# smpurkis/PyTorch-Face-Detection-from-Scratch

Hardware: AMD Instinct MI355X
Metric: train imgs/sec (PoolResnet 480^2, bs=256 per GPU) (higher is better)
Workload: dtype f32 (3x3 convs: bf16x3 split MFMA, fp32 accumulate)

## Files before the change

### pytorch-face-detection-from-scratch_amd/csrc/fdet_wgrad3x3_ps.hip

```cpp
#include "fdet_conv3x3_x3.h"
#include "fdet_ps.h"
#include "fdet_ldsdma.h"
#include <algorithm>

using namespace fdet;

typedef __attribute__((address_space(3))) void* lds_void_t;
typedef const __attribute__((address_space(1))) void* glb_void_t;
typedef short s16x4 __attribute__((ext_vector_type(4)));
typedef __attribute__((address_space(3))) s16x4* lds_s16x4_t;
typedef __bf16 bf16x2_t __attribute__((ext_vector_type(2)));
typedef unsigned u32x2_t __attribute__((ext_vector_type(2)));
typedef unsigned u32x4_t __attribute__((ext_vector_type(4)));

namespace {

#ifndef WG_DBG
#define WG_DBG 0
#endif
constexpr int WG_MAXL = 16;
constexpr int XL = 5, ZL = 3;
constexpr int XA = XL * 64 + 4;
constexpr int ZLS = 66;
constexpr int ZA = 212;
constexpr int WG_LDS_UNITS = 16 * XA + 16 * ZA;

struct PsWgArgs {
  const bf16x8* x[WG_MAXL];
  const bf16x8* dz[WG_MAXL];
  float* ws;
  float* wsb;
  int plane, img;
  int lpi, real_lpi, nlines;
  int nslab, lpw;
  unsigned magic_lpi;
};

__device__ __forceinline__ bf16x2_t as_bf16x2(unsigned u) { return __builtin_bit_cast(bf16x2_t, u); }
__device__ __forceinline__ u32x2_t tr2(const char* base, int off) {
  return __builtin_bit_cast(u32x2_t, __builtin_amdgcn_ds_read_tr16_b64_v4i16((lds_s16x4_t)(base + off)));
}
__host__ __device__ constexpr int x_line(int S, int ky, int WP) { return 16 * S + (ky - 1) * WP < 0 ? 0 : (16 * S + (ky - 1) * WP >= 64 ? 2 : 1); }
__host__ __device__ constexpr int x_off(int S, int ky, int WP) {
  return 16 * S + (ky - 1) * WP < 0 ? 16 * S + (ky - 1) * WP + 64 : (16 * S + (ky - 1) * WP >= 64 ? 16 * S + (ky - 1) * WP - 64 : 16 * S + (ky - 1) * WP);
}

template <int WP, bool FL1, bool P16 = false>
__global__ void __launch_bounds__(256, 1)
k_wgrad3x3_ps(const PsWgArgs a) {
  extern __shared__ __attribute__((aligned(16))) char smem[];
  bf16x8* const lds = reinterpret_cast<bf16x8*>(smem);
  const int tid = threadIdx.x, lane = tid & 63;
  const int wid = __builtin_amdgcn_readfirstlane(tid >> 6);
  const int m = wid & 1, j = wid >> 1;
  const int layer = blockIdx.y;
  const bf16x8* __restrict__ gx = a.x[layer];
  const bf16x8* __restrict__ gz = a.dz[layer];
  {
    f32x4* z = reinterpret_cast<f32x4*>(smem);
    for (int t = tid; t < WG_LDS_UNITS; t += 256) z[t] = f32x4{0.f, 0.f, 0.f, 0.f};
  }
  const int i16 = lane & 15, g16 = (lane >> 4) & 1, kh = lane >> 5;
  const int q = i16 >> 2, pp = i16 & 3;
  const int GA = 4 * m + 2 * g16 + (pp >> 1), GB = 4 * j + 2 * g16 + (pp >> 1);
  const int lane_x = (GB * XA + 8 * kh + q) * 16 + (pp & 1) * 8;
  const int lane_z = (16 * XA + GA * ZA + 1 + 8 * kh + q) * 16 + (pp & 1) * 8;
  constexpr int XPL = 8 * XA * 16, ZPL = 8 * ZA * 16;

  const int l0 = blockIdx.x * a.lpw, l1 = min(l0 + a.lpw, a.nlines);
  f32x16 acc[9];
#pragma unroll
  for (int t = 0; t < 9; ++t)
#pragma unroll
    for (int r = 0; r < 16; ++r) acc[t][r] = 0.f;
  float bsum = 0.f;
  const unsigned bsel0 = j == 0 ? 0x3f803f80u : 0u, bsel1 = j == 1 ? 0x3f803f80u : 0u;

  const unsigned lds0 = (unsigned)(size_t)(lds_void_t)smem;
  const unsigned tbytes = (unsigned)((a.nlines / a.lpi) + 2) * (unsigned)a.img * 16u;
  const dma_u32x4 xrs = dma_rsrc(gx - a.img, tbytes), zrs = dma_rsrc(gz - a.img, tbytes);
  const unsigned lane16 = (unsigned)lane * 16u;
#define WG_PIECE(RS, LG, AI, DST)                                                                  \
  {                                                                                                \
    const int lg_ = (LG) + a.lpi;                                                                  \
    const int n_ = (int)__umulhi((unsigned)lg_, a.magic_lpi);                                      \
    const unsigned so_ = (unsigned)(n_ * a.img + ((AI) >> 3) * a.plane + ((AI) & 7) * (a.lpi * 64) + (lg_ - n_ * a.lpi) * 64) * 16u; \
    dma_piece(lds0 + (unsigned)(DST) * 16u, lane16, RS, so_);                                      \
  }
#define WG_ISSUE(LX, SX, LZ, SZ)                                                                   \
  if (!(P16 && wid >= 2)) {                                   \
    _Pragma("unroll") for (int k_ = 0; k_ < 4; ++k_) {                                             \
      const int ai_ = 4 * wid + k_;                                                                \
      WG_PIECE(xrs, LX, ai_, ai_ * XA + (SX) * 64)                                                  \
      WG_PIECE(zrs, LZ, ai_, 16 * XA + ai_ * ZA + (SZ) * ZLS + 1)                                   \
    }                                                                                              \
  }
  __syncthreads();
  int sx = ((l0 - 1) % XL + XL) % XL, sz = l0 % ZL;
#define XS(D) ((sx + (D)) % XL)
  WG_ISSUE(l0 - 1, XS(0), l0, sz)
  WG_ISSUE(l0, XS(1), l0 + 1, (sz + 1) % ZL)
  if (!(P16 && wid >= 2)) {
    _Pragma("unroll") for (int k_ = 0; k_ < 4; ++k_) {
      const int ai_ = 4 * wid + k_;
      WG_PIECE(xrs, l0 + 1, ai_, ai_ * XA + XS(2) * 64)
      WG_PIECE(xrs, l0 + 2, ai_, ai_ * XA + XS(3) * 64)
    }
  }
  asm volatile("s_waitcnt vmcnt(0)" ::: "memory");

  u32x4_t zf[2][3][2], xf[2][3][2];
#define WG_FRAGS(F, S, ZB, XB0, XB1, XB2)                                                          \
  {                                                                                                \
    _Pragma("unroll") for (int k_ = 0; k_ < 3; ++k_)                                               \
      _Pragma("unroll") for (int pl_ = 0; pl_ < (P16 ? 1 : 2); ++pl_)                              \
        _Pragma("unroll") for (int h_ = 0; h_ < 2; ++h_) {                                         \
          const u32x2_t z_ = (WG_DBG & 4) ? u32x2_t{0x3f803f80u + (unsigned)lane, 0x40004000u} : tr2(ZB, pl_ * ZPL + (16 * (S) + 4 * h_ - (k_ - 1)) * 16); \
          zf[F][k_][pl_][2 * h_] = z_[0]; zf[F][k_][pl_][2 * h_ + 1] = z_[1];                      \
          const char* xb_ = x_line((S), k_, WP) == 0 ? XB0 : (x_line((S), k_, WP) == 1 ? XB1 : XB2); \
          const u32x2_t x_ = (WG_DBG & 4) ? u32x2_t{0x3f803f80u, 0x40004000u + (unsigned)lane} : tr2(xb_, pl_ * XPL + (x_off((S), k_, WP) + 4 * h_) * 16); \
          xf[F][k_][pl_][2 * h_] = x_[0]; xf[F][k_][pl_][2 * h_ + 1] = x_[1];                      \
        }                                                                                          \
  }
  int band = l0;
  if (FL1) {
    __builtin_amdgcn_s_barrier();
    const char* zb_ = smem + lane_z + sz * (ZLS * 16);
    const char* xb0 = smem + lane_x + XS(0) * 1024;
    const char* xb1 = smem + lane_x + XS(1) * 1024;
    const char* xb2 = smem + lane_x + XS(2) * 1024;
    WG_FRAGS(0, 0, zb_, xb0, xb1, xb2)
  }
  int row = l0 - (l0 / a.lpi) * a.lpi;
  while (band < l1) {
  const int n_full = row < a.real_lpi ? min(l1 - band, a.real_lpi - row) : 0;
  row += n_full;
  for (const int bend = band + n_full; band < bend; ++band) {
    if (FL1) asm volatile("s_waitcnt vmcnt(0)" ::: "memory");
    else asm volatile("s_waitcnt vmcnt(8)" ::: "memory");
    __builtin_amdgcn_s_barrier();
    if (!(WG_DBG & 1)) WG_ISSUE(band + 3, XS(4), band + 2, (sz + 2) % ZL)
    __builtin_amdgcn_sched_barrier(0);
    {
      const char* zb_ = smem + lane_z + sz * (ZLS * 16);
      const char* xb0 = smem + lane_x + XS(0) * 1024;
      const char* xb1 = smem + lane_x + XS(1) * 1024;
      const char* xb2 = smem + lane_x + XS(2) * 1024;
      const char* zbn = smem + lane_z + ((sz + 1) % ZL) * (ZLS * 16);
      const char* xb3 = smem + lane_x + XS(3) * 1024;
      if (!FL1) {
        WG_FRAGS(0, 0, zb_, xb0, xb1, xb2)
        __builtin_amdgcn_sched_barrier(0);
      }
#pragma unroll
      for (int s = 0; s < 4; ++s) {
        const int F = s & 1;
        if (s < 3) WG_FRAGS(F ^ 1, s + 1, zb_, xb0, xb1, xb2)
        else if (FL1) WG_FRAGS(0, 0, zbn, xb1, xb2, xb3)
#pragma unroll
        for (int ky = 0; ky < 3; ++ky)
#pragma unroll
          for (int kx = 0; kx < 3; ++kx) {
            const int t = ky * 3 + kx;
            const bf16x8 ah = __builtin_bit_cast(bf16x8, zf[F][kx][0]), al = __builtin_bit_cast(bf16x8, zf[F][kx][1]);
            const bf16x8 bh = __builtin_bit_cast(bf16x8, xf[F][ky][0]), bl = __builtin_bit_cast(bf16x8, xf[F][ky][1]);
            if (!(WG_DBG & 2)) {
              if (!P16) {
                acc[t] = __builtin_amdgcn_mfma_f32_32x32x16_bf16(ah, bl, acc[t], 0, 0, 0);
                acc[t] = __builtin_amdgcn_mfma_f32_32x32x16_bf16(al, bh, acc[t], 0, 0, 0);
              }
              acc[t] = __builtin_amdgcn_mfma_f32_32x32x16_bf16(ah, bh, acc[t], 0, 0, 0);
            }
          }
        {
          const bf16x2_t sel = as_bf16x2((s & 1) ? bsel1 : bsel0);
#pragma unroll
          for (int pl = 0; pl < (P16 ? 1 : 2); ++pl) {
            const u32x4_t zv = zf[F][1][pl];
            bsum = __builtin_amdgcn_fdot2_f32_bf16(as_bf16x2(zv[0]), sel, bsum, false);
            bsum = __builtin_amdgcn_fdot2_f32_bf16(as_bf16x2(zv[1]), sel, bsum, false);
            bsum = __builtin_amdgcn_fdot2_f32_bf16(as_bf16x2(zv[2]), sel, bsum, false);
            bsum = __builtin_amdgcn_fdot2_f32_bf16(as_bf16x2(zv[3]), sel, bsum, false);
          }
        }
        if ((s < 3 || FL1) && !P16) {
#pragma unroll
          for (int i = 0; i < 24; ++i) {
            __builtin_amdgcn_sched_group_barrier(0x008, 1, 0);
            __builtin_amdgcn_sched_group_barrier(0x100, 1, 0);
          }
          __builtin_amdgcn_sched_group_barrier(0x008, 3, 0);
        } else if (s < 3 || FL1) {
#pragma unroll
          for (int i = 0; i < 9; ++i) {
            __builtin_amdgcn_sched_group_barrier(0x008, 1, 0);
            if (i < 6) __builtin_amdgcn_sched_group_barrier(0x100, 2, 0);
          }
        }
      }
    }
    sx = (sx + 1) % XL;
    sz = (sz + 1) % ZL;
  }
  if (band < l1 && row >= a.real_lpi) {
    const int n_zero = min(l1 - band, a.lpi - row);
    for (const int bend = band + n_zero; band < bend; ++band) {
      asm volatile("s_waitcnt vmcnt(0)" ::: "memory");
      __builtin_amdgcn_s_barrier();
      if (!(WG_DBG & 1)) WG_ISSUE(band + 3, XS(4), band + 2, (sz + 2) % ZL)
      sx = (sx + 1) % XL;
      sz = (sz + 1) % ZL;
    }
    row += n_zero;
    if (row >= a.lpi) row = 0;
    if (FL1 && band < l1) {
      const char* zb_ = smem + lane_z + sz * (ZLS * 16);
      const char* xb0 = smem + lane_x + XS(0) * 1024;
      const char* xb1 = smem + lane_x + XS(1) * 1024;
      const char* xb2 = smem + lane_x + XS(2) * 1024;
      WG_FRAGS(0, 0, zb_, xb0, xb1, xb2)
    }
  }
  }
  asm volatile("s_waitcnt vmcnt(0)" ::: "memory");
#undef WG_FRAGS
#undef XS
#undef WG_ISSUE
#undef WG_PIECE
  const int l31 = lane & 31, half = lane >> 5;
  const size_t s = (size_t)layer * a.nslab + blockIdx.x;
  float* __restrict__ wsl = a.ws + s * 9 * 64 * 64;
#pragma unroll
  for (int t = 0; t < 9; ++t)
#pragma unroll
    for (int r = 0; r < 16; ++r) {
      const int co = 32 * m + (r & 3) + 8 * (r >> 2) + 4 * half;
      wsl[(t * 64 + co) * 64 + 32 * j + l31] = acc[t][r];
    }
  bsum += __shfl_xor(bsum, 32, 64);
  if (half == 0) a.wsb[(s * 2 + j) * 64 + 32 * m + l31] = bsum;
}

struct PsWgRed { float* dW[WG_MAXL]; float* db[WG_MAXL]; };
__global__ void __launch_bounds__(256)
k_wgrad_ps_reduce(const float* __restrict__ ws, const float* __restrict__ wsb, int nslab, const PsWgRed out) {
  __shared__ float part[256];
  const int layer = blockIdx.y;
  const int el = threadIdx.x & 63, q = threadIdx.x >> 6;
  const bool bias_blk = blockIdx.x == 9 * 64;
  const size_t stride = bias_blk ? 128 : 9 * 4096;
  const float* __restrict__ src = bias_blk ? wsb + (size_t)layer * nslab * 128 + el
                                           : ws + (size_t)layer * nslab * 9 * 4096 + (size_t)blockIdx.x * 64 + el;
  float s = 0.f;
  int k = q;
  for (; k + 28 < nslab; k += 32) {
    float v[8];
#pragma unroll
    for (int u = 0; u < 8; ++u) v[u] = src[(size_t)(k + 4 * u) * stride] + (bias_blk ? src[(size_t)(k + 4 * u) * stride + 64] : 0.f);
#pragma unroll
    for (int u = 0; u < 8; ++u) s += v[u];
  }
  for (; k < nslab; k += 4) s += src[(size_t)k * stride] + (bias_blk ? src[(size_t)k * stride + 64] : 0.f);
  part[threadIdx.x] = s;
  __syncthreads();
  if (q == 0) {
    const float r = ((part[el] + part[64 + el]) + part[128 + el]) + part[192 + el];
    if (bias_blk) {
      out.db[layer][el] = r;
    } else {
      const int e = blockIdx.x * 64 + el;
      const int t = e >> 12, co = (e >> 6) & 63, ci = e & 63;
      out.dW[layer][(co * 64 + ci) * 9 + t] = r;
    }
  }
}

int wg_plan(int L, int N, int H, int W, PsGeo& g, int& nslab, int& lpw) {
  PsStrips sp;
  if (!ps_geo_strips(N, 64, H, W, g, sp) || L < 1 || L > WG_MAXL) return 0;
  const int lpi = g.HP * g.WP / 64;
  const long nlines = (long)g.N * lpi;
  if (nlines + 2 * lpi >= (1 << 20) || (size_t)(g.N + 2) * g.img * 16 >= ((size_t)1 << 32)) return 0;
  nslab = std::max(1, std::min((int)nlines, num_cus() / L));
  lpw = (int)((nlines + nslab - 1) / nslab);
  nslab = (int)((nlines + lpw - 1) / lpw);
  return 1;
}

}

extern "C" size_t fdet_conv3x3_wgrad_ps_ws_bytes(int L, int N, int C, int H, int W) {
  PsGeo g;
  int nslab = 0, lpw = 0;
  if (C != 64 || !wg_plan(L, N, H, W, g, nslab, lpw)) return 0;
  return (size_t)L * nslab * (9 * 4096 + 128) * sizeof(float);
}

namespace {
int wgrad_ps_run(const void* const* h_x, const void* const* h_dz, float* const* h_dW, float* const* h_db, int L, int N, int C,
                 int H, int W, void* ws, size_t ws_bytes, void* stream, bool p16) {
  PsGeo g;
  int nslab = 0, lpw = 0;
  FDET_REQUIRE(h_x && h_dz && h_dW && h_db && ws, "conv3x3_wgrad_ps: null pointer");
  FDET_REQUIRE(C == 64 && wg_plan(L, N, H, W, g, nslab, lpw), "conv3x3_wgrad_ps: unsupported shape (L=%d N=%d C=%d H=%d W=%d)", L, N, C, H, W);
  const size_t need = (size_t)L * nslab * (9 * 4096 + 128) * sizeof(float);
  FDET_REQUIRE(ws_bytes >= need, "conv3x3_wgrad_ps: workspace of %zu bytes needed, %zu given", need, ws_bytes);
  PsWgArgs a;
  PsWgRed red;
  for (int l = 0; l < L; ++l) {
    FDET_REQUIRE(h_x[l] && h_dz[l] && h_dW[l] && h_db[l], "conv3x3_wgrad_ps: null pointer in layer %d", l);
    a.x[l] = reinterpret_cast<const bf16x8*>(h_x[l]);
    a.dz[l] = reinterpret_cast<const bf16x8*>(h_dz[l]);
    red.dW[l] = h_dW[l];
    red.db[l] = h_db[l];
  }
  a.ws = reinterpret_cast<float*>(ws);
  a.wsb = a.ws + (size_t)L * nslab * 9 * 4096;
  a.plane = g.plane; a.img = g.img;
  a.lpi = g.HP * g.WP / 64;
  a.real_lpi = (H * g.WP + 63) / 64;
  a.nlines = g.N * a.lpi;
  a.nslab = nslab; a.lpw = lpw;
  a.magic_lpi = magic_of(a.lpi);
  const size_t lds = (size_t)WG_LDS_UNITS * 16;
  hipStream_t st = (hipStream_t)stream;
  static const bool fl1 = [] { const char* e = getenv("FDET_WGPS_FLIGHT"); return !(e && e[0] == '2'); }();
  auto go = [&](auto kern, bool& done) -> int {
    if (!done) {
      if (hipFuncSetAttribute((const void*)kern, hipFuncAttributeMaxDynamicSharedMemorySize, (int)lds) != hipSuccess) {
        (void)hipGetLastError();
        return fail(FDET_ELAUNCH, "conv3x3_wgrad_ps: cannot reserve %zu bytes of LDS", lds);
      }
      done = true;
    }
    hipLaunchKernelGGL(kern, dim3(nslab, L), dim3(256), lds, st, a);
    return FDET_OK;
  };
  static bool d64a = false, d64b = false, d32a = false, d32b = false, d16a = false, d16b = false, d64p = false, d32p = false, d16p = false;
  int rc0;
  if (p16) {
    if (g.WP == 64) rc0 = go(k_wgrad3x3_ps<64, true, true>, d64p);
    else if (g.WP == 16) rc0 = go(k_wgrad3x3_ps<16, true, true>, d16p);
    else rc0 = go(k_wgrad3x3_ps<32, true, true>, d32p);
  }
  else if (g.WP == 64) rc0 = fl1 ? go(k_wgrad3x3_ps<64, true>, d64a) : go(k_wgrad3x3_ps<64, false>, d64b);
  else if (g.WP == 16) rc0 = fl1 ? go(k_wgrad3x3_ps<16, true>, d16a) : go(k_wgrad3x3_ps<16, false>, d16b);
  else rc0 = fl1 ? go(k_wgrad3x3_ps<32, true>, d32a) : go(k_wgrad3x3_ps<32, false>, d32b);
  if (rc0 != FDET_OK) return rc0;
  int rc = check_launch("fdet_conv3x3_wgrad_ps_batched");
  if (rc != FDET_OK) return rc;
  hipLaunchKernelGGL(k_wgrad_ps_reduce, dim3(9 * 64 + 1, L), dim3(256), 0, st, a.ws, a.wsb, nslab, red);
  return check_launch("fdet_conv3x3_wgrad_ps_batched(reduce)");
}
}

extern "C" int fdet_conv3x3_wgrad_ps_batched(const void* const* h_x, const void* const* h_dz, float* const* h_dW,
                                             float* const* h_db, int L, int N, int C, int H, int W, void* ws,
                                             size_t ws_bytes, void* stream) {
  return wgrad_ps_run(h_x, h_dz, h_dW, h_db, L, N, C, H, W, ws, ws_bytes, stream, false);
}

extern "C" int fdet_conv3x3_wgrad_ps_batched_p16(const void* const* h_x, const void* const* h_dz, float* const* h_dW,
                                                 float* const* h_db, int L, int N, int C, int H, int W, void* ws,
                                                 size_t ws_bytes, void* stream) {
  return wgrad_ps_run(h_x, h_dz, h_dW, h_db, L, N, C, H, W, ws, ws_bytes, stream, true);
}
```

Measured before the change: 93860.

## Interleave wgrad DMA issues with MFMA taps and strength-reduce ring addressing

Result: no change. 94430, median of 6 (+0.6%).

```diff
diff --git a/pytorch-face-detection-from-scratch_amd/csrc/fdet_wgrad3x3_ps.hip b/pytorch-face-detection-from-scratch_amd/csrc/fdet_wgrad3x3_ps.hip
--- a/pytorch-face-detection-from-scratch_amd/csrc/fdet_wgrad3x3_ps.hip
+++ b/pytorch-face-detection-from-scratch_amd/csrc/fdet_wgrad3x3_ps.hip
@@ -17,6 +17,9 @@
 
 #ifndef WG_DBG
 #define WG_DBG 0
+#endif
+#ifndef WG_PLACE
+#define WG_PLACE 1
 #endif
 constexpr int WG_MAXL = 16;
 constexpr int XL = 5, ZL = 3;
@@ -40,6 +43,7 @@
 __device__ __forceinline__ u32x2_t tr2(const char* base, int off) {
   return __builtin_bit_cast(u32x2_t, __builtin_amdgcn_ds_read_tr16_b64_v4i16((lds_s16x4_t)(base + off)));
 }
+__device__ __forceinline__ int ring_add(int v, int d, int lim) { const int t = v + d; return t >= lim ? t - lim : t; }
 __host__ __device__ constexpr int x_line(int S, int ky, int WP) { return 16 * S + (ky - 1) * WP < 0 ? 0 : (16 * S + (ky - 1) * WP >= 64 ? 2 : 1); }
 __host__ __device__ constexpr int x_off(int S, int ky, int WP) {
   return 16 * S + (ky - 1) * WP < 0 ? 16 * S + (ky - 1) * WP + 64 : (16 * S + (ky - 1) * WP >= 64 ? 16 * S + (ky - 1) * WP - 64 : 16 * S + (ky - 1) * WP);
@@ -80,55 +84,120 @@
   const unsigned tbytes = (unsigned)((a.nlines / a.lpi) + 2) * (unsigned)a.img * 16u;
   const dma_u32x4 xrs = dma_rsrc(gx - a.img, tbytes), zrs = dma_rsrc(gz - a.img, tbytes);
   const unsigned lane16 = (unsigned)lane * 16u;
-#define WG_PIECE(RS, LG, AI, DST)                                                                  \
-  {                                                                                                \
-    const int lg_ = (LG) + a.lpi;                                                                  \
-    const int n_ = (int)__umulhi((unsigned)lg_, a.magic_lpi);                                      \
-    const unsigned so_ = (unsigned)(n_ * a.img + ((AI) >> 3) * a.plane + ((AI) & 7) * (a.lpi * 64) + (lg_ - n_ * a.lpi) * 64) * 16u; \
-    dma_piece(lds0 + (unsigned)(DST) * 16u, lane16, RS, so_);                                      \
-  }
-#define WG_ISSUE(LX, SX, LZ, SZ)                                                                   \
+  unsigned arr_src[4], arr_x[4], arr_z[4];
+#pragma unroll
+  for (int k = 0; k < 4; ++k) {
+    const int ai = 4 * wid + k;
+    arr_src[k] = (unsigned)((ai >> 3) * a.plane + (ai & 7) * (a.lpi * 64)) * 16u;
+    arr_x[k] = lds0 + (unsigned)(ai * XA) * 16u;
+    arr_z[k] = lds0 + (unsigned)(16 * XA + ai * ZA + 1) * 16u;
+  }
+  auto line_off = [&](int LG) -> unsigned {
+    const int lg = LG + a.lpi;
+    const int n = (int)__umulhi((unsigned)lg, a.magic_lpi);
+    return (unsigned)(n * a.img + (lg - n * a.lpi) * 64) * 16u;
+  };
+#define WG_PIECE(P, LBX, SBX, LBZ, SBZ)                                                            \
+  {                                                                                                \
+    if ((P) & 1) dma_piece(arr_z[(P) >> 1] + (unsigned)(SBZ), lane16, zrs, (LBZ) + arr_src[(P) >> 1]); \
+    else dma_piece(arr_x[(P) >> 1] + (unsigned)(SBX), lane16, xrs, (LBX) + arr_src[(P) >> 1]);     \
+  }
+#define WG_ISSUE(LBX, SBX, LBZ, SBZ)                                                               \
   if (!(P16 && wid >= 2)) {                                   \
-    _Pragma("unroll") for (int k_ = 0; k_ < 4; ++k_) {                                             \
-      const int ai_ = 4 * wid + k_;                                                                \
-      WG_PIECE(xrs, LX, ai_, ai_ * XA + (SX) * 64)                                                  \
-      WG_PIECE(zrs, LZ, ai_, 16 * XA + ai_ * ZA + (SZ) * ZLS + 1)                                   \
+    _Pragma("unroll") for (int p_ = 0; p_ < 8; ++p_) WG_PIECE(p_, LBX, SBX, LBZ, SBZ)              \
+  }
+  __syncthreads();
+  constexpr int XSB = 1024, ZSB = ZLS * 16;
+  int sxb = (((l0 - 1) % XL + XL) % XL) * XSB, szb = (l0 % ZL) * ZSB;
+#define XS(D) ring_add(sxb, (D) * XSB, XL * XSB)
+#define ZS(D) ring_add(szb, (D) * ZSB, ZL * ZSB)
+  {
+    const unsigned o0 = line_off(l0 - 1), o1 = line_off(l0), o2 = line_off(l0 + 1), o3 = line_off(l0 + 2);
+    WG_ISSUE(o0, XS(0), o1, ZS(0))
+    WG_ISSUE(o1, XS(1), o2, ZS(1))
+    if (!(P16 && wid >= 2)) {
+      _Pragma("unroll") for (int k_ = 0; k_ < 4; ++k_) {
+        WG_PIECE(2 * k_, o2, XS(2), 0u, 0)
+        WG_PIECE(2 * k_, o3, XS(3), 0u, 0)
+      }
+    }
+  }
+  asm volatile("s_waitcnt vmcnt(0)" ::: "memory");
+  unsigned lbx = line_off(l0 + 3), lbz = line_off(l0 + 2);
+  int rwx;
+  {
+    const int lg = l0 + 3 + a.lpi;
+    rwx = lg - (int)__umulhi((unsigned)lg, a.magic_lpi) * a.lpi;
+  }
+  const unsigned img_skip = (unsigned)(a.img - a.lpi * 64) * 16u;
+  int xfill = XS(4), zfill = ZS(2);
+  const char* zb_ = smem + lane_z + ZS(0);
+  const char* zbn = smem + lane_z + ZS(1);
+  const char* xb0 = smem + lane_x + XS(0);
+  const char* xb1 = smem + lane_x + XS(1);
+  const char* xb2 = smem + lane_x + XS(2);
+  const char* xb3 = smem + lane_x + XS(3);
+#define WG_ADVANCE                                                                                 \
+  {                                                                                                \
+    zb_ = zbn; zbn = smem + lane_z + zfill;                                                        \
+    xb0 = xb1; xb1 = xb2; xb2 = xb3; xb3 = smem + lane_x + xfill;                                  \
+    xfill = sxb; zfill = szb;                                                                      \
+    sxb = XS(1); szb = ZS(1);                                                                      \
+    if (!(WG_DBG & 8)) {                                                                           \
+      lbz = lbx;                                                                                   \
+      const bool wrap_ = ++rwx == a.lpi;                                                           \
+      lbx += wrap_ ? 1024u + img_skip : 1024u;                                                     \
+      rwx = wrap_ ? 0 : rwx;                                                                       \
     }                                                                                              \
   }
-  __syncthreads();
-  int sx = ((l0 - 1) % XL + XL) % XL, sz = l0 % ZL;
-#define XS(D) ((sx + (D)) % XL)
-  WG_ISSUE(l0 - 1, XS(0), l0, sz)
-  WG_ISSUE(l0, XS(1), l0 + 1, (sz + 1) % ZL)
-  if (!(P16 && wid >= 2)) {
-    _Pragma("unroll") for (int k_ = 0; k_ < 4; ++k_) {
-      const int ai_ = 4 * wid + k_;
-      WG_PIECE(xrs, l0 + 1, ai_, ai_ * XA + XS(2) * 64)
-      WG_PIECE(xrs, l0 + 2, ai_, ai_ * XA + XS(3) * 64)
-    }
-  }
-  asm volatile("s_waitcnt vmcnt(0)" ::: "memory");
 
   u32x4_t zf[2][3][2], xf[2][3][2];
+  constexpr int NFR = P16 ? 12 : 24;
+#define WG_FRAG1(F, S, I, ZB, XB0, XB1, XB2)                                                       \
+  {                                                                                                \
+    const int h_ = ((I) >> 1) & 1, pl_ = P16 ? 0 : ((I) >> 2) & 1, k_ = (I) >> (P16 ? 2 : 3);      \
+    if (((I) & 1) == 0) {                                                                          \
+      const u32x2_t z_ = (WG_DBG & 4) ? u32x2_t{0x3f803f80u + (unsigned)lane, 0x40004000u} : tr2(ZB, pl_ * ZPL + (16 * (S) + 4 * h_ - (k_ - 1)) * 16); \
+      zf[F][k_][pl_][2 * h_] = z_[0]; zf[F][k_][pl_][2 * h_ + 1] = z_[1];                          \
+    } else {                                                                                       \
+      const char* xb_ = x_line((S), k_, WP) == 0 ? XB0 : (x_line((S), k_, WP) == 1 ? XB1 : XB2);   \
+      const u32x2_t x_ = (WG_DBG & 4) ? u32x2_t{0x3f803f80u, 0x40004000u + (unsigned)lane} : tr2(xb_, pl_ * XPL + (x_off((S), k_, WP) + 4 * h_) * 16); \
+      xf[F][k_][pl_][2 * h_] = x_[0]; xf[F][k_][pl_][2 * h_ + 1] = x_[1];                          \
+    }                                                                                              \
+  }
 #define WG_FRAGS(F, S, ZB, XB0, XB1, XB2)                                                          \
   {                                                                                                \
-    _Pragma("unroll") for (int k_ = 0; k_ < 3; ++k_)                                               \
-      _Pragma("unroll") for (int pl_ = 0; pl_ < (P16 ? 1 : 2); ++pl_)                              \
-        _Pragma("unroll") for (int h_ = 0; h_ < 2; ++h_) {                                         \
-          const u32x2_t z_ = (WG_DBG & 4) ? u32x2_t{0x3f803f80u + (unsigned)lane, 0x40004000u} : tr2(ZB, pl_ * ZPL + (16 * (S) + 4 * h_ - (k_ - 1)) * 16); \
-          zf[F][k_][pl_][2 * h_] = z_[0]; zf[F][k_][pl_][2 * h_ + 1] = z_[1];                      \
-          const char* xb_ = x_line((S), k_, WP) == 0 ? XB0 : (x_line((S), k_, WP) == 1 ? XB1 : XB2); \
-          const u32x2_t x_ = (WG_DBG & 4) ? u32x2_t{0x3f803f80u, 0x40004000u + (unsigned)lane} : tr2(xb_, pl_ * XPL + (x_off((S), k_, WP) + 4 * h_) * 16); \
-          xf[F][k_][pl_][2 * h_] = x_[0]; xf[F][k_][pl_][2 * h_ + 1] = x_[1];                      \
-        }                                                                                          \
-  }
+    _Pragma("unroll") for (int i_ = 0; i_ < NFR; ++i_) WG_FRAG1(F, S, i_, ZB, XB0, XB1, XB2)       \
+  }
+#define WG_TAP(F, T)                                                                               \
+  {                                                                                                \
+    const int ky_ = (T) / 3, kx_ = (T) % 3;                                                        \
+    const bf16x8 ah = __builtin_bit_cast(bf16x8, zf[F][kx_][0]), al = __builtin_bit_cast(bf16x8, zf[F][kx_][1]); \
+    const bf16x8 bh = __builtin_bit_cast(bf16x8, xf[F][ky_][0]), bl = __builtin_bit_cast(bf16x8, xf[F][ky_][1]); \
+    if (!(WG_DBG & 2)) {                                                                           \
+      if (!P16) {                                                                                  \
+        acc[T] = __builtin_amdgcn_mfma_f32_32x32x16_bf16(ah, bl, acc[T], 0, 0, 0);                 \
+        acc[T] = __builtin_amdgcn_mfma_f32_32x32x16_bf16(al, bh, acc[T], 0, 0, 0);                 \
+      }                                                                                            \
+      acc[T] = __builtin_amdgcn_mfma_f32_32x32x16_bf16(ah, bh, acc[T], 0, 0, 0);                   \
+    }                                                                                              \
+  }
+#define WG_BIAS(F, S)                                                                              \
+  {                                                                                                \
+    const bf16x2_t sel = as_bf16x2(((S) & 1) ? bsel1 : bsel0);                                     \
+    _Pragma("unroll") for (int pl = 0; pl < (P16 ? 1 : 2); ++pl) {                                 \
+      const u32x4_t zv = zf[F][1][pl];                                                             \
+      bsum = __builtin_amdgcn_fdot2_f32_bf16(as_bf16x2(zv[0]), sel, bsum, false);                  \
+      bsum = __builtin_amdgcn_fdot2_f32_bf16(as_bf16x2(zv[1]), sel, bsum, false);                  \
+      bsum = __builtin_amdgcn_fdot2_f32_bf16(as_bf16x2(zv[2]), sel, bsum, false);                  \
+      bsum = __builtin_amdgcn_fdot2_f32_bf16(as_bf16x2(zv[3]), sel, bsum, false);                  \
+    }                                                                                              \
+  }
+  constexpr bool PLACED = FL1 && !P16 && WG_PLACE != 0;
+  constexpr int NCARRY = WG_PLACE == 2 ? 2 : 1, GAP = WG_PLACE == 2 ? 2 : 1;
   int band = l0;
   if (FL1) {
     __builtin_amdgcn_s_barrier();
-    const char* zb_ = smem + lane_z + sz * (ZLS * 16);
-    const char* xb0 = smem + lane_x + XS(0) * 1024;
-    const char* xb1 = smem + lane_x + XS(1) * 1024;
-    const char* xb2 = smem + lane_x + XS(2) * 1024;
     WG_FRAGS(0, 0, zb_, xb0, xb1, xb2)
   }
   int row = l0 - (l0 / a.lpi) * a.lpi;
@@ -139,15 +208,9 @@
     if (FL1) asm volatile("s_waitcnt vmcnt(0)" ::: "memory");
     else asm volatile("s_waitcnt vmcnt(8)" ::: "memory");
     __builtin_amdgcn_s_barrier();
-    if (!(WG_DBG & 1)) WG_ISSUE(band + 3, XS(4), band + 2, (sz + 2) % ZL)
+    if (!PLACED && !(WG_DBG & 1)) WG_ISSUE(lbx, xfill, lbz, zfill)
     __builtin_amdgcn_sched_barrier(0);
     {
-      const char* zb_ = smem + lane_z + sz * (ZLS * 16);
-      const char* xb0 = smem + lane_x + XS(0) * 1024;
-      const char* xb1 = smem + lane_x + XS(1) * 1024;
-      const char* xb2 = smem + lane_x + XS(2) * 1024;
-      const char* zbn = smem + lane_z + ((sz + 1) % ZL) * (ZLS * 16);
-      const char* xb3 = smem + lane_x + XS(3) * 1024;
       if (!FL1) {
         WG_FRAGS(0, 0, zb_, xb0, xb1, xb2)
         __builtin_amdgcn_sched_barrier(0);
@@ -155,34 +218,32 @@
 #pragma unroll
       for (int s = 0; s < 4; ++s) {
         const int F = s & 1;
+        if (PLACED && s < NCARRY) {
+#pragma unroll
+          for (int t = 0; t < 9; ++t) {
+#pragma unroll
+            for (int i = 3 * t; i < 3 * t + 3; ++i)
+              if (i < NFR) WG_FRAG1(F ^ 1, s + 1, i, zb_, xb0, xb1, xb2)
+            WG_TAP(F, t)
+#pragma unroll
+            for (int i = 3 * t; i < 3 * t + 3; ++i) {
+              __builtin_amdgcn_sched_group_barrier(0x008, 1, 0);
+              if (i < NFR) __builtin_amdgcn_sched_group_barrier(0x100, 1, 0);
+            }
+            if ((t + 1) % GAP == 0 && (t + 1) / GAP <= 8 / NCARRY) {
+              __builtin_amdgcn_sched_barrier(0);
+              if (!(WG_DBG & 1)) WG_PIECE(s * (8 / NCARRY) + (t + 1) / GAP - 1, lbx, xfill, lbz, zfill)
+              __builtin_amdgcn_sched_barrier(0);
+            }
+          }
+          WG_BIAS(F, s)
+          continue;
+        }
         if (s < 3) WG_FRAGS(F ^ 1, s + 1, zb_, xb0, xb1, xb2)
         else if (FL1) WG_FRAGS(0, 0, zbn, xb1, xb2, xb3)
 #pragma unroll
-        for (int ky = 0; ky < 3; ++ky)
-#pragma unroll
-          for (int kx = 0; kx < 3; ++kx) {
-            const int t = ky * 3 + kx;
-            const bf16x8 ah = __builtin_bit_cast(bf16x8, zf[F][kx][0]), al = __builtin_bit_cast(bf16x8, zf[F][kx][1]);
-            const bf16x8 bh = __builtin_bit_cast(bf16x8, xf[F][ky][0]), bl = __builtin_bit_cast(bf16x8, xf[F][ky][1]);
-            if (!(WG_DBG & 2)) {
-              if (!P16) {
-                acc[t] = __builtin_amdgcn_mfma_f32_32x32x16_bf16(ah, bl, acc[t], 0, 0, 0);
-                acc[t] = __builtin_amdgcn_mfma_f32_32x32x16_bf16(al, bh, acc[t], 0, 0, 0);
-              }
-              acc[t] = __builtin_amdgcn_mfma_f32_32x32x16_bf16(ah, bh, acc[t], 0, 0, 0);
-            }
-          }
-        {
-          const bf16x2_t sel = as_bf16x2((s & 1) ? bsel1 : bsel0);
-#pragma unroll
-          for (int pl = 0; pl < (P16 ? 1 : 2); ++pl) {
-            const u32x4_t zv = zf[F][1][pl];
-            bsum = __builtin_amdgcn_fdot2_f32_bf16(as_bf16x2(zv[0]), sel, bsum, false);
-            bsum = __builtin_amdgcn_fdot2_f32_bf16(as_bf16x2(zv[1]), sel, bsum, false);
-            bsum = __builtin_amdgcn_fdot2_f32_bf16(as_bf16x2(zv[2]), sel, bsum, false);
-            bsum = __builtin_amdgcn_fdot2_f32_bf16(as_bf16x2(zv[3]), sel, bsum, false);
-          }
-        }
+        for (int t = 0; t < 9; ++t) WG_TAP(F, t)
+        WG_BIAS(F, s)
         if ((s < 3 || FL1) && !P16) {
 #pragma unroll
           for (int i = 0; i < 24; ++i) {
@@ -199,31 +260,30 @@
         }
       }
     }
-    sx = (sx + 1) % XL;
-    sz = (sz + 1) % ZL;
+    WG_ADVANCE
   }
   if (band < l1 && row >= a.real_lpi) {
     const int n_zero = min(l1 - band, a.lpi - row);
     for (const int bend = band + n_zero; band < bend; ++band) {
       asm volatile("s_waitcnt vmcnt(0)" ::: "memory");
       __builtin_amdgcn_s_barrier();
-      if (!(WG_DBG & 1)) WG_ISSUE(band + 3, XS(4), band + 2, (sz + 2) % ZL)
-      sx = (sx + 1) % XL;
-      sz = (sz + 1) % ZL;
+      if (!(WG_DBG & 1)) WG_ISSUE(lbx, xfill, lbz, zfill)
+      WG_ADVANCE
     }
     row += n_zero;
     if (row >= a.lpi) row = 0;
     if (FL1 && band < l1) {
-      const char* zb_ = smem + lane_z + sz * (ZLS * 16);
-      const char* xb0 = smem + lane_x + XS(0) * 1024;
-      const char* xb1 = smem + lane_x + XS(1) * 1024;
-      const char* xb2 = smem + lane_x + XS(2) * 1024;
       WG_FRAGS(0, 0, zb_, xb0, xb1, xb2)
     }
   }
   }
   asm volatile("s_waitcnt vmcnt(0)" ::: "memory");
+#undef WG_BIAS
+#undef WG_TAP
 #undef WG_FRAGS
+#undef WG_FRAG1
+#undef WG_ADVANCE
+#undef ZS
 #undef XS
 #undef WG_ISSUE
 #undef WG_PIECE
@@ -233,9 +293,9 @@
 #pragma unroll
   for (int t = 0; t < 9; ++t)
 #pragma unroll
-    for (int r = 0; r < 16; ++r) {
-      const int co = 32 * m + (r & 3) + 8 * (r >> 2) + 4 * half;
-      wsl[(t * 64 + co) * 64 + 32 * j + l31] = acc[t][r];
+    for (int g = 0; g < 4; ++g) {
+      const int co = 32 * m + 8 * g + 4 * half;
+      *reinterpret_cast<f32x4*>(wsl + (t * 64 + 32 * j + l31) * 64 + co) = f32x4{acc[t][4 * g], acc[t][4 * g + 1], acc[t][4 * g + 2], acc[t][4 * g + 3]};
     }
   bsum += __shfl_xor(bsum, 32, 64);
   if (half == 0) a.wsb[(s * 2 + j) * 64 + 32 * m + l31] = bsum;
@@ -269,7 +329,7 @@
       out.db[layer][el] = r;
     } else {
       const int e = blockIdx.x * 64 + el;
-      const int t = e >> 12, co = (e >> 6) & 63, ci = e & 63;
+      const int t = e >> 12, ci = (e >> 6) & 63, co = e & 63;
       out.dW[layer][(co * 64 + ci) * 9 + t] = r;
     }
   }
@@ -305,6 +365,7 @@
   FDET_REQUIRE(C == 64 && wg_plan(L, N, H, W, g, nslab, lpw), "conv3x3_wgrad_ps: unsupported shape (L=%d N=%d C=%d H=%d W=%d)", L, N, C, H, W);
   const size_t need = (size_t)L * nslab * (9 * 4096 + 128) * sizeof(float);
   FDET_REQUIRE(ws_bytes >= need, "conv3x3_wgrad_ps: workspace of %zu bytes needed, %zu given", need, ws_bytes);
+  FDET_REQUIRE(((size_t)ws & 15) == 0, "conv3x3_wgrad_ps: the workspace must be 16-byte aligned");
   PsWgArgs a;
   PsWgRed red;
   for (int l = 0; l < L; ++l) {
```
